# ishine/usdm

Hardware: AMD Instinct MI355X
Metric: end-to-end real-time factor + LLM tokens/sec, 10 s utterance, 7B TP=1/8 (higher is better)
Workload: dtype bf16; 1 GPU; full pipeline, one 10 s utterance: XLS-R tokenizer -> Mistral-7B (3 greedy rounds) -> Token-Voicebox 63 NFE (Heun, CFG, 3 s prompt) -> BigVGAN; wave_samples=160000, mel_frames=861, output_samples=220416, parallelism=tp1 (LLM) + replicas, tp_comm=none, voicebox=replica (CFG batch 2 on every rank)

## Files before the change

### include/usdm_hip.h

```cpp
#ifndef USDM_HIP_H_
#define USDM_HIP_H_
#include <stdint.h>

#ifdef __cplusplus
extern "C" {
#endif

typedef void* usdm_stream_t;

enum { USDM_BF16 = 0, USDM_F32 = 1 };
enum { USDM_ACT_NONE = 0, USDM_ACT_GELU = 1, USDM_ACT_SWIGLU = 3, USDM_ACT_TANH = 4, USDM_ACT_LOGCLAMP = 5  };
enum { USDM_EPI_PLAIN = 0, USDM_EPI_QKV_HEADS = 1 };

const char* usdm_last_error(void);
int usdm_abi_version(void);

typedef struct usdm_gemm_args {
  int32_t dtype;
  int32_t M, N;
  int32_t taps, Kc;
  const void* A;
  int64_t lda;
  int32_t rowsA;
  int32_t a_row_mul, a_row_off, a_row_step;
// ... 177 lines not shown
int usdm_sizeof_gemv_mxfp4_args(void);

typedef struct usdm_gemv_mxfp4_mfma_args {
  usdm_gemv_batch_args b;
  const void* codes;
  int64_t ldc;
  const uint8_t* scales;
  int64_t lds;
} usdm_gemv_mxfp4_mfma_args;
int usdm_gemv_mxfp4_mfma(const usdm_gemv_mxfp4_mfma_args* args, usdm_stream_t stream);
int usdm_sizeof_gemv_mxfp4_mfma_args(void);

typedef struct usdm_gemv_wpack {
  const void* planes;
  const uint8_t* rowflag;
  int64_t stride;
  int32_t base;
  int32_t units;
  uint32_t marked[448];
} usdm_gemv_wpack;
int usdm_gemv_packed(const usdm_gemv_args* args, const usdm_gemv_wpack* pack, usdm_stream_t stream);
int usdm_gemv_packs(const usdm_gemv_args* args);
int usdm_sizeof_gemv_wpack(void);

typedef struct usdm_decode_state {
  int32_t* next_token;
  int32_t* out_tokens;
  int32_t* step;
  int32_t* pos;
  int32_t max_out, id_offset, advance_pos;
  int32_t batch;
  int32_t* done; const int32_t* eos;
} usdm_decode_state;
int usdm_argmax_final(const float* part_val, const int32_t* part_idx, int32_t nparts,
                      const usdm_decode_state* st, const void* embed_table_bf16, int32_t Hd, void* h_out_bf16,
                      usdm_stream_t stream);
int usdm_argmax_final_seg(const float* part_val, const int32_t* part_idx, int32_t nparts, int32_t nseg, int64_t seg_stride,
                          const usdm_decode_state* st, const void* embed_table, int32_t Hd, void* h_out, usdm_stream_t stream);

typedef struct usdm_sample_params {
  float temperature; int32_t top_k; float top_p;
  float min_p;
  uint64_t seed;
} usdm_sample_params;
typedef struct usdm_sample_args {
  const float* logits; int32_t V;
// ... 244 lines not shown
```

### usdm_amd/_lib.py

```python
import ctypes as C
import os

_HERE = os.path.dirname(os.path.abspath(__file__))
LIB_PATH = os.path.join(_HERE, "libusdm_hip.so")


class UsdmError(RuntimeError):
    pass


if not os.path.exists(LIB_PATH):
    raise ImportError(
        f"{LIB_PATH} not found: build it with `python -m usdm_amd.build` (hipcc --offload-arch=gfx950). "
        "usdm_amd has no CPU fallback.")

lib = C.CDLL(LIB_PATH, mode=C.RTLD_GLOBAL)
lib.usdm_last_error.restype = C.c_char_p
lib.usdm_gemv_batch_ks_floats.restype = C.c_int64
lib.usdm_gemm_tile_info.restype = C.c_int
lib.usdm_gemv_fp8_mfma.restype = C.c_int
lib.usdm_attn_decode_fp8.restype = C.c_int
lib.usdm_rope_cache_fp8.restype = C.c_int
lib.usdm_gemv_mxfp4.restype = C.c_int
lib.usdm_dequant_mxfp4.restype = C.c_int
lib.usdm_gemv_mxfp4_mfma.restype = C.c_int
lib.usdm_gemv_packed.restype = C.c_int
lib.usdm_gemv_packs.restype = C.c_int
lib.usdm_logprobs.restype = C.c_int
lib.usdm_logprobs_seg.restype = C.c_int
lib.usdm_prompt_logprobs.restype = C.c_int
lib.usdm_prompt_logprobs_seg.restype = C.c_int
lib.usdm_penalize.restype = C.c_int
lib.usdm_penalize_seg.restype = C.c_int
lib.usdm_penalty_params_init.restype = C.c_int
lib.usdm_logit_edit.restype = C.c_int
lib.usdm_logit_edit_seg.restype = C.c_int
lib.usdm_beam_step.restype = C.c_int
lib.usdm_kv_reorder.restype = C.c_int
lib.usdm_kv_expand.restype = C.c_int
lib.usdm_attn_verify.restype = C.c_int
lib.usdm_spec_commit.restype = C.c_int
lib.usdm_attn_verify_batch.restype = C.c_int
lib.usdm_spec_commit_batch.restype = C.c_int
_exp = None


def exp():
    global _exp
    if _exp is None:
        path = os.path.join(_HERE, "libusdm_hip_experimental.so")
# ... 313 lines not shown
```

### usdm_amd/csrc/llm_k.hip

```cpp
#include "common.h"
#include <stdlib.h>
#include <utility>
#include "../../include/usdm_hip.h"
#include "gemv_launch.h"
#include "gemv_pieces.h"
#include "attn_merge.h"
#include "p2p.h"
#include "pick_commit.h"

#ifndef USDM_GEMV_DOWN_UNR
#define USDM_GEMV_DOWN_UNR 8
#endif
#ifndef USDM_GEMV_WPACK_RU
#define USDM_GEMV_WPACK_RU 3
#endif
#ifndef USDM_GEMV_WPACK_UB
#define USDM_GEMV_WPACK_UB 12
#endif
namespace {
#ifdef USDM_GEMV_TRACE
__device__ unsigned long long g_gemv_trace[8192 * 8];
#define GTR(i) do { if (threadIdx.x == 0 && blockIdx.x < 8192) g_gemv_trace[blockIdx.x * 8 + (i)] = wall_clock64(); } while (0)
#else
#define GTR(i) do { } while (0)
#endif


template <int RW, bool GLU, int NWV, bool MRG = false, bool P2P = false, bool CMB = false, bool FP8 = false, class... FMT>
__global__ __launch_bounds__(NWV * 64) void gemv_kernel(const usdm_gemv_args a, FMT... fmt) {
  typedef typename gemv_fmt<FP8>::wvec wvec;
  constexpr bool MX4 = gemv_is_mx4<FMT...>::value;
  static_assert((FP8 || MX4) == (sizeof...(FMT) == 1) && !(FP8 && MX4), "FP8 takes the row exponents, MXFP4 the block scales");
  static_assert(!(FP8 || MX4) || (!MRG && !P2P && !CMB), "the FP8 / MXFP4 weight formats have the plain single-GPU forms only");
  constexpr int NTH = NWV * 64;
  constexpr int NR = GLU ? 2 * RW : RW;
  constexpr int UNR = gemv_ring_depth(NR, FP8, MX4);
  extern __shared__ __attribute__((aligned(16))) char smem[];
  bf16_t* xs = (bf16_t*)smem;
  __shared__ float red[NWV];
  __shared__ float sv[NWV];
// ... 606 lines not shown
    gemv_for<NU>([&](auto UI) {
      constexpr int un = decltype(UI)::value, s = un % RU;
      constexpr int younger = un + RU < NU ? 4 * (RU - 1) : 4 * (NU - 1 - un);
      gemv_wunit& r = ring[s];
      asm volatile("s_waitcnt vmcnt(%4)" : "+v"(r.la), "+v"(r.lb), "+v"(r.nib), "+v"(r.sgn) : "n"(younger) : "memory");
      gemv_for<4>([&](auto PI) {
        constexpr int P = decltype(PI)::value, it = 4 * un + P;
        const u32x4 xn = *(const u32x4*)(xs + (((it + 1) % NIT) * 64 + lane) * 8);
        const u32x4& lo = P < 2 ? r.la : r.lb;
        acc = dot8(gemv_wpack8<P>(lo[2 * (P & 1)], lo[2 * (P & 1) + 1], r.nib[P], r.sgn, base4), xv, acc);
        xv = xn;
      });
      if constexpr (un + RU < NU) gemv_unit_load<un + RU>(r, pp, voff);
    });
  }
  acc = wave_sum(acc);

  if (lane != 0 || ob >= a.N) return;
  const float v = gemv_plain_value(acc, a.round_bf16, a.residual != nullptr, [&] { return bf2f(resraw); });
  if (a.y16) ((bf16_t*)a.y16)[ob] = f2bf(v);
  if (a.y32) a.y32[ob] = v;
}

__global__ void argmax_final_kernel(const float* pv, const int* pi, int nparts, int nseg, int64_t seg_stride, usdm_decode_state st,
                                    const bf16_t* E, int Hd, bf16_t* h_out) {
  __shared__ float sv[256];
  __shared__ int si[256];
  __shared__ int s_tok;
  const int b = blockIdx.x;
  if (st.done && st.done[b]) return;
  pv += (int64_t)b * nparts; pi += (int64_t)b * nparts;
  float bv = -INFINITY;
  int bi = PICK_NO_ID;
  for (int sg = 0; sg < nseg; ++sg)
    for (int i = threadIdx.x; i < nparts; i += 256) {
      const float v = pv[sg * seg_stride + i];
      const int id = pi[sg * seg_stride + i];
      if (pick_better(v, id, bv, bi)) { bv = v; bi = id; }
    }
  pick_block_best<256>(sv, si, bv, bi);
  if (threadIdx.x == 0) {
    const int tok = (si[0] == PICK_NO_ID ? 0 : si[0]) + st.id_offset;
    pick_commit(st, b, st.step[b], tok);
    s_tok = tok;
  }
  if (E) {
    __syncthreads();
    pick_embed_row<256>(E, s_tok, Hd, h_out + (int64_t)b * Hd);
  }
}

__global__ void embed_kernel(const bf16_t* E, const int64_t* ids, const int* next_token, int n, int Hd, bf16_t* out) {
  const int r = blockIdx.x;
  const int64_t id = ids ? ids[r] : (int64_t)(*next_token);
  const u32x4* src = (const u32x4*)(E + id * Hd);
  u32x4* dst = (u32x4*)(out + (int64_t)r * Hd);
  for (int i = threadIdx.x; i < Hd / 8; i += blockDim.x) dst[i] = src[i];
}

__global__ void residual_add_kernel(bf16_t* h, const float* delta, int n) {
  const int i = blockIdx.x * blockDim.x + threadIdx.x;
  if (i < n) h[i] = f2bf(bf2f(h[i]) + round_bf(delta[i]));
}
}

static int gemv_resident_count(const void* kern, int nth, size_t lds, int* out) {
  static thread_local const void* c_kern = nullptr;
  static thread_local int c_dev = -1, c_n = 0;
  static thread_local size_t c_lds = 0;
  int dev = 0;
  USDM_HIP(hipGetDevice(&dev));
  if (kern != c_kern || dev != c_dev || lds != c_lds) {
    int ncu = 0, per = 0;
    USDM_HIP(hipDeviceGetAttribute(&ncu, hipDeviceAttributeMultiprocessorCount, dev));
    USDM_HIP(hipOccupancyMaxActiveBlocksPerMultiprocessor(&per, kern, nth, lds));
    USDM_CHECK_ARG(ncu > 0 && per > 0, "usdm_gemv: the resident form does not fit a CU (%zu bytes of LDS)", lds);
    c_kern = kern; c_dev = dev; c_lds = lds; c_n = ncu * per;
  }
  *out = c_n;
  return 0;
}

static int gemv_launch_resident(const usdm_gemv_args& a, const gemv_sel& s, size_t lds, hipStream_t st, bool* launched) {
  *launched = false;
  if (a.x_delta) return 0;
  constexpr int RW = 2, NWV = 7;
  auto straight = gemv_resident_kernel<RW, NWV, 2, 8>;
  auto generic = gemv_resident_kernel<RW, NWV, 0, 0>;
  const int ntiles = s.grid;
  int n = 0;
  if (int rc = gemv_resident_count((const void*)straight, NWV * 64, lds, &n)) return rc;
  int grid = min(min(n, s.res), ntiles);
  if (grid == ntiles) return 0;
  if (a.K == 8 * 512 && ntiles == 2 * grid) {
    hipLaunchKernelGGL(straight, dim3(grid), dim3(NWV * 64), lds, st, a);
  } else {
    if (int rc = gemv_resident_count((const void*)generic, NWV * 64, lds, &n)) return rc;
    grid = min(min(n, s.res), ntiles);
    if (grid == ntiles) return 0;
    hipLaunchKernelGGL(generic, dim3(grid), dim3(NWV * 64), lds, st, a);
  }
  *launched = true;
  USDM_LAUNCH_CHECK();
  return 0;
}

template <int FORM, bool MRG, bool P2P, bool CMB, bool FP8, class... FMT>
static int gemv_launch(const usdm_gemv_args& a, hipStream_t st, FMT... fmt) {
  const size_t lds = (size_t)((a.K + 511) & ~511) * 2;
  const gemv_sel s = gemv_select(a, false);
  if constexpr (FORM == GEMV_PLAIN && !FP8 && sizeof...(FMT) == 0) {
    if (s.stream) {
      hipLaunchKernelGGL((gemv_stream_kernel<28, USDM_GEMV_DOWN_UNR>), dim3(s.grid), dim3(1024), lds, st, a);
      USDM_LAUNCH_CHECK();
      return 0;
    }
    if (s.res > 0) {
// ... 41 lines not shown
  }
  return gemv_launch<GEMV_PLAIN, false, false, false, false>(a, st);
}

extern "C" int usdm_gemv_packs(const usdm_gemv_args* pa) { return gemv_select(*pa, false).stream ? 1 : 0; }

extern "C" int usdm_gemv_packed(const usdm_gemv_args* pa, const usdm_gemv_wpack* pk, usdm_stream_t stream) {
  USDM_CHECK_ARG(pa && pa->W && pa->x && pk && pk->planes && pk->rowflag, "usdm_gemv_packed: null args");
  USDM_CHECK_ARG(pa->N <= 14336, "usdm_gemv_packed: at most 14336 rows (usdm_gemv_wpack.marked)");
  if (!usdm_gemv_packs(pa)) return usdm_gemv(pa, stream);
  const usdm_gemv_args& a = *pa;
  if (int rc = gemv_check_shape("usdm_gemv_packed", a, "input vector")) return rc;
  if (int rc = gemv_check_outputs("usdm_gemv_packed", a)) return rc;
  USDM_CHECK_ARG(pk->units == 7 && pk->units * 2048 == a.K && pk->stride % 16 == 0 && pk->stride >= (int64_t)pk->units * GEMV_WPACK_UNIT &&
                     pk->base >= 0 && pk->base <= 112,
                 "usdm_gemv_packed: the image must hold K / 2048 units of 3328 bytes per row, stride a multiple of 16, base 0..112");
  USDM_CHECK_ARG(((uintptr_t)pk->planes & 15) == 0 && ((uintptr_t)pk->rowflag & 3) == 0, "usdm_gemv_packed: planes must be 16-byte, rowflag 4-byte aligned");
  const gemv_sel s = gemv_select(a, false);
  hipLaunchKernelGGL((gemv_stream_wpack_kernel<28, USDM_GEMV_WPACK_RU, USDM_GEMV_WPACK_UB>), dim3(s.grid), dim3(1024), (size_t)a.K * 2,
                     (hipStream_t)stream, a, *pk);
  USDM_LAUNCH_CHECK();
  return 0;
}
extern "C" int usdm_sizeof_gemv_wpack(void) { return (int)sizeof(usdm_gemv_wpack); }

int usdm_gemv_fp8_batch_launch(const usdm_gemv_fp8_args* pa, hipStream_t st);

extern "C" int usdm_gemv_fp8(const usdm_gemv_fp8_args* pa, usdm_stream_t stream) {
  USDM_CHECK_ARG(pa && pa->b.g.W && pa->b.g.x && pa->row_exp, "usdm_gemv_fp8: null args");
  const usdm_gemv_args& a = pa->b.g;
  USDM_CHECK_ARG(pa->b.nb >= 1 && pa->b.nb <= 4 && (pa->b.form == 0 || pa->b.form == -1),
                 "usdm_gemv_fp8: 1..4 sequences on the VALU form (the matrix-core form has no FP8 weights)");
  USDM_CHECK_ARG(!a.p2p && !a.p2p_mode && !a.mrg_po && !a.cmb_gran && !a.x_delta && !a.x_out,
                 "usdm_gemv_fp8: p2p / merged-attention input / cmb_gran / x_delta are not supported with FP8 weights");
  USDM_CHECK_ARG(((uintptr_t)a.W & 7) == 0, "usdm_gemv_fp8: bad N/K/ldw");
  if (int rc = gemv_check_shape("usdm_gemv_fp8", a, "input vector")) return rc;
  if (int rc = gemv_check_outputs("usdm_gemv_fp8", a)) return rc;
  hipStream_t st = (hipStream_t)stream;
  if (pa->b.nb > 1) return usdm_gemv_fp8_batch_launch(pa, st);
  return gemv_launch<GEMV_PLAIN, false, false, false, true>(a, st, pa->row_exp);
}

namespace {
__global__ __launch_bounds__(256) void dequant_fp8_kernel(const uint8_t* q, const int8_t* row_exp, int K, int64_t ldq, bf16_t* out,
                                                          int64_t ldo) {
  const int r = blockIdx.x;
// ... 128 lines not shown
```

### usdm_amd/llm.py

```python
import math
import os
import time
from collections import namedtuple

import torch

from . import ops
from ._lib import ACT_SWIGLU, UsdmError
from .graph import GraphedPlan, GraphedSegments
from .plancache import LRU
from .prefix import reusable_past
from .quant import Fp8Weight, Mxfp4Weight, check_kv_cache_dtype
from .wpack import PackedWeight
from .slots import (CHUNK, NO_CANDIDATE_IDX, BeamSlots, DecodeSlots, SpecSequence, SpecSlots, TokenLogprobs, edit_buffers, logprob_buffers,
                    penalty_buffers, read_logprobs, seed_edits, seed_penalties, stop_block, stop_index)

MISTRAL_7B_USDM = dict(vocab_size=42003, hidden_size=4096, intermediate_size=14336, num_hidden_layers=32,
                       num_attention_heads=32, num_key_value_heads=8, head_dim=128, rms_norm_eps=1e-5,
                       rope_theta=10000.0, max_position_embeddings=32768)


def _pack_gate_up(gate, up):
    I, K = gate.shape
    return torch.stack([gate.reshape(I // 16, 16, K), up.reshape(I // 16, 16, K)], 1).reshape(2 * I, K).contiguous()
# ... 139 lines not shown
         "lm_head": qz_head(g("lm_head.weight")[v0:v1].contiguous()), "layers": [], "v0": v0, "v1": v1}
    for l in range(cfg["num_hidden_layers"]):
        p = f"model.layers.{l}."
        q = g(p + "self_attn.q_proj.weight")[rank * Hq * d:(rank + 1) * Hq * d]
        k = g(p + "self_attn.k_proj.weight")[rank * Hkv * d:(rank + 1) * Hkv * d]
        v = g(p + "self_attn.v_proj.weight")[rank * Hkv * d:(rank + 1) * Hkv * d]
        o = g(p + "self_attn.o_proj.weight")[:, rank * Hq * d:(rank + 1) * Hq * d]
        ga = g(p + "mlp.gate_proj.weight")[rank * I:(rank + 1) * I]
        up = g(p + "mlp.up_proj.weight")[rank * I:(rank + 1) * I]
        dn = g(p + "mlp.down_proj.weight")[:, rank * I:(rank + 1) * I]
        W["layers"].append(dict(qkv=qz(torch.cat([q, k, v], 0).contiguous()), o=qz(o.contiguous()), gu=qz(_pack_gate_up(ga, up)),
                                down=qz(dn.contiguous()), ln1=f(p + "input_layernorm.weight"),
                                ln2=f(p + "post_attention_layernorm.weight")))
        del q, k, v, o, ga, up, dn
    return W


class USDMForCausalLM:
    def __init__(self, cfg, device, ctx_max=2048, tp_rank=0, tp_size=1, group=None, decode_splits=None, tp_segments=None, p2p=None,
                 p2p_fused=None, quantization=None, fp8_matrix_cores=False, kv_cache_dtype=None, score_rows=256,
                 enable_prefix_caching=False, weight_packing=None, mxfp4_matrix_cores=False):
        check_quantization(quantization, fp8_matrix_cores, mxfp4_matrix_cores)
        self.weight_packing = (os.environ.get("USDM_WPACK", "1") != "0") if weight_packing is None else bool(weight_packing)
        self.wpack_report = None
        self.prefix_caching = bool(enable_prefix_caching)
        if self.prefix_caching:
            if tp_size > 1 or tp_segments or p2p is not None:
                raise NotImplementedError("enable_prefix_caching runs on one GPU: tensor parallelism (tp_size > 1, tp_segments, p2p) is not supported")
            if os.environ.get("USDM_PREFIX_REUSE", "exact") in ("0", "off"):
                raise ValueError("enable_prefix_caching=True contradicts USDM_PREFIX_REUSE=0 (prefix reuse switched off)")
        if isinstance(score_rows, bool) or not isinstance(score_rows, int) or score_rows < 16 or score_rows % 16:
            raise ValueError(f"score_rows must be a positive multiple of 16, got {score_rows!r}")
        self.score_rows = score_rows
        if quantization is not None and (tp_size > 1 or tp_segments or p2p is not None):
            raise NotImplementedError(f"quantization={quantization!r} runs on one GPU: tensor parallelism (tp_size > 1, tp_segments, p2p) takes bf16 weights")
        self.kv_cache_dtype = check_kv_cache_dtype(kv_cache_dtype)
        self.kv8 = self.kv_cache_dtype == "fp8"
        if self.kv8 and (tp_size > 1 or tp_segments or p2p is not None):
            raise NotImplementedError("kv_cache_dtype='fp8' runs on one GPU: tensor parallelism (tp_size > 1, tp_segments, p2p) takes a bf16 cache")
        if self.kv8 and os.environ.get("USDM_GEMV_CHAIN", "0") not in ("", "0"):
            raise NotImplementedError("kv_cache_dtype='fp8': the chained decode GEMVs (USDM_GEMV_CHAIN) take a bf16 cache")
        self.quantization = quantization
        self.fp8_matrix_cores = bool(fp8_matrix_cores)
        self.mxfp4_matrix_cores = bool(mxfp4_matrix_cores)
        self.cfg = dict(cfg)
        self.device = torch.device(device)
# ... 127 lines not shown
                           p + "mlp.gate_proj.weight": ((I, H), H ** -0.5), p + "mlp.up_proj.weight": ((I, H), H ** -0.5),
                           p + "mlp.down_proj.weight": ((H, I), I ** -0.5)})

        def get(n):
            if n.endswith("norm.weight") or n.endswith("layernorm.weight"):
                return torch.ones(H, device=m.device)
            shape, sc = shapes[n]
            return (torch.randn(shape, device=m.device, dtype=torch.float32, generator=gen) * sc).to(torch.bfloat16)
        m.W = m._shard(get)
        m._alloc()
        return m

    def weight_bytes_per_token(self):
        if self.quantization is not None:
            return sum(l[k].nbytes for l in self.W["layers"] for k in QUANT_KEYS) + self.W["lm_head"].nbytes
        n = sum(l[k].numel() for l in self.W["layers"] for k in ("qkv", "o", "gu", "down")) + self.W["lm_head"].numel()
        return 2 * n

    def kv_bytes_per_token_row(self):
        d = self.cfg["head_dim"]
        return 2 * self.cfg["num_hidden_layers"] * self.Hkv * ((d + 1) if self.kv8 else 2 * d)

    def _pack_weights(self):
        self.wpack_down = None
        if not (self.weight_packing and self.tp_size == 1 and not self.tp_path and self.p2p is None and self.quantization is None
                and self.cfg["hidden_size"] == 4096 and self.I == 14336):
            return
        t0 = time.perf_counter()
        self.wpack_down = [PackedWeight.from_matrix(w["down"]) for w in self.W["layers"]]
        torch.cuda.synchronize(self.device)
        self.wpack_report = {"down_marked_share": [p.marked_share for p in self.wpack_down],
                             "down_marked_rows": sum(len(p.marked_rows) for p in self.wpack_down),
                             "extra_bytes": sum(p.nbytes for p in self.wpack_down), "seconds": time.perf_counter() - t0}

    def _alloc(self):
        self._pack_weights()
        c, dev = self.cfg, self.device
        L, d = c["num_hidden_layers"], c["head_dim"]
        bf = torch.bfloat16
        if self.kv8:
            self.kcache = torch.zeros(L, self.Hkv, self.ctx_max, d, dtype=torch.uint8, device=dev)
            self.vcache = torch.zeros(L, self.Hkv, self.ctx_max, d, dtype=torch.uint8, device=dev)
            self.kexp = torch.zeros(L, self.Hkv, self.ctx_max, dtype=torch.int8, device=dev)
            self.vexp = torch.zeros(L, self.Hkv, self.ctx_max, dtype=torch.int8, device=dev)
        else:
            self.kcache = torch.zeros(L, self.Hkv, self.ctx_max, d, dtype=bf, device=dev)
            self.vcache = torch.zeros(L, self.Hkv, self.ctx_max, d, dtype=bf, device=dev)
        mode = os.environ.get("USDM_PREFIX_REUSE", "exact")
        self.reuse_prefix = {"0": False, "off": False, "1": True, "all": True}.get(mode, "exact")
        if self.kv8:
            self.vtc = None
            if not self.prefix_caching:
                self.reuse_prefix = False
        else:
            self.vtc = torch.zeros(L, self.Hkv, d, self.ctx_max, dtype=bf, device=dev)
        self._kv_ids, self._vt_upto = None, 0
# ... 149 lines not shown
                ops.penalize(logits, st, V=self.v1 - self.v0, plan=rec.plan, **pen)
            if sampling == "hook":
                rec.cut(lambda: self.logits_hook())
            ops.sample_final(logits, st, dev_params=sl.sample_params, plan=rec.plan, **out)
            if lp:
                ops.logprobs(logits, st, V=self.v1 - self.v0, plan=rec.plan, **lp)
        elif p2p is not None:
            site = 2 * c["num_hidden_layers"]
            self._p2p_exchange(rec, st, lambda ph: ops.argmax_p2p(sl.part_val_loc, sl.part_idx_loc, self.nparts, st, p2p, site, phase=ph,
                                                                  plan=rec.plan, **out))
        else:
            if self.tp_path:
                rec.cut(self._gather_partials if single else
                        (lambda: self._gather_partials([sl.part_val, sl.part_idx], [sl.part_val_loc, sl.part_idx_loc])))
            seg = dict(nseg=self.tp_size, seg_stride=B * self.nparts) if (B and self.tp_path) else {}
            ops.argmax_final(sl.part_val, sl.part_idx, self.nparts * (1 if B else self.tp_size), st, plan=rec.plan, **seg, **out)
        rec.plan.hold(st)

    def _dims(self):
        c = self.cfg
        H, d = c["hidden_size"], c["head_dim"]
        return H, d, c["num_hidden_layers"], self.Hq, self.Hkv, self.I, (self.Hq + 2 * self.Hkv) * d

    def _layers(self, rec, gemv, attn, h, qkv, ao, act, way, n=0, parts=None, h_alt=None, down_kw={}, down_wp=None):
        H, d, _, Hq, Hkv, I, nq = self._dims()
        eps, h0, pend = self.cfg["rms_norm_eps"], h, None

        def proj(W, ln, N, out, a=0):
            nonlocal h, pend
            if pend is None:
                return gemv(W, h, N=N, K=H, norm_w=ln, eps=eps, act=a, y16=out)
            nxt = h_alt if h is h0 else h0
            gemv(W, h, N=N, K=H, norm_w=ln, eps=eps, act=a, y16=out, x_delta=pend, x_out=nxt)
            h, pend = nxt, None

        def land(W, x, K, site, **kw):
            nonlocal pend
            if way == "fused":
                return gemv(W, x, N=H, K=K, residual=h, y16=h, **kw)
            if way == "p2p":
                mode = 1 if self.p2p_fused else 2
                gemv(W, x, N=H, K=K, residual=h, y16=h, p2p=self.p2p, p2p_site=site, p2p_mode=mode, **kw)
                rec.cut()
                if mode == 2:
                    ops.p2p_reduce(self.p2p, site, H, h, skip=self.st_done, plan=rec.plan)
                return
            part = parts[site & 1]
            gemv(W, x, N=H, K=K, round_bf16=False, y32=part, **kw)
            rec.cut(lambda: self._all_reduce(part))
            if way == "deferred":
                pend = part
            else:
                ops.residual_add(h, part, n, plan=rec.plan)

        for l, w in enumerate(self.W["layers"]):
            proj(w["qkv"], w["ln1"], nq, qkv)
            o_kw = attn(l) or {}
            land(w["o"], ao, Hq * d, 2 * l, **o_kw)
            proj(w["gu"], w["ln2"], 2 * I, act, ACT_SWIGLU)
            land(w["down"], act, I, 2 * l + 1, **down_kw, **({"wpack": down_wp[l]} if down_wp else {}))
        return h, pend

    def _prefill_rows(self, S, slot=None, past=0):
        dev, bf = self.device, torch.bfloat16
        H, d, L, Hq, Hkv, I, nq = self._dims()
        scratch = slot is not None or self.kv8
        Spad = ((past if scratch else 0) + S + 63) // 64 * 64
        rec = _Segments()
        Z = lambda *s, dt=bf: rec.plan.hold(torch.zeros(*s, device=dev, dtype=dt))
        io = dict(ids=Z(S, dt=torch.int64))
        h, xn, qkv, ao, act = Z(S, H), Z(S, H), Z(S, nq), Z(S, Hq * d), Z(S, I)
        vt = Z(Hkv, d, Spad) if scratch else None
        kscr = Z(Hkv, Spad, d) if self.kv8 else None
        part = Z(S, H, dt=torch.float32) if self.tp_path else None
        ops.embed_rows(self.W["embed"], h, Hd=H, ids=io["ids"], n=S, plan=rec.plan)

        def gemm(W, x, *, N, K, norm_w=None, eps=None, act=0, residual=None, y16=None, y32=None, round_bf16=True):
            if norm_w is not None:
                ops.norm(x, norm_w, None, rows=S, C=H, eps=eps, rms=True, round_bf16=True, out16=xn, plan=rec.plan)
                x = xn
            ops.gemm(x, self._gemm_w(W, rec.plan), M=S, N=N, Kc=K, act=act, round_bf16=round_bf16 and (bool(act) or residual is not None),
                     residual=residual, ldr=H if residual is not None else 0, out32=y32, out16=y16, ldc=N // 2 if act else N, plan=rec.plan)
# ... 97 lines not shown
            else:
                ops.gemv_chain(chain, sync, plan=rec.plan)
            chain = None

        def gemv(W, x, **kw):
            if chain is None:
                return ops.gemv(W, x, skip=skp, plan=rec.plan, **kw)
            chain.append(ops.gemv(W, x, skip=skp, only_args=True, **kw))
            if len(chain) == self.chain:
                flush()

        def attn(l):
            nonlocal chain
            gran = cmb_gran[l] if use_cmb else None
            ops.attn_decode(qkv, self.st_pos, self.cos, self.sin, self.kcache[l], self.vcache[l], pm, pl, po, ao, Hq=Hq, Hkv=Hkv,
                            ctx_max=self.ctx_max, NS=self.NS, scale=d ** -0.5, counters=cnt, skip=skp, defer_merge=mrg is not None, window=self.window,
                            cmb_gran=gran, kv8=(self.kexp[l], self.vexp[l]) if self.kv8 else None, plan=rec.plan)
            if chained:
                chain = []
                return None
            return dict(merge=mrg, cmb=(gran, self.cmb_err) if use_cmb else None)

        h, pend = self._layers(rec, gemv, attn, h, qkv, ao, act, way, n=H, parts=parts, h_alt=h_alt,
                               down_wp=self.wpack_down if way == "fused" else None)
        if chain:
            flush()
        self._lm_head_and_pick(rec, h, True, sampling, x_delta=pend, skip=skp, logprobs=logprobs, penalties=penalties, edits=edits)
        return rec.finish()

    @staticmethod
    def _run_segs(segs):
        for s in segs:
            if isinstance(s, ops.Plan):
                s.run()
            else:
                s()

    def _graphed(self, built, enabled=None):
        segs = built if isinstance(built, list) else [built]
        if any(not isinstance(s, ops.Plan) for s in segs):
            return GraphedSegments(segs, self._run_segs, enabled=enabled)
        plan = segs[0]
        if len(segs) > 1:
            plan = ops.Plan()
            for s in segs:
                plan.calls += s.calls
                plan.hold(*s.keep)
# ... 510 lines not shown
```

### usdm_amd/ops.py

```python
import ctypes as C_
import os

import torch

from . import _lib
from ._lib import (BF16, F32, AttnVerifyArgs, AttnVerifyBatchArgs, SpecArgs, SpecBatchArgs, BeamArgs, KvExpandArgs, KvReorderArgs, AttnArgs, AttnDecodeArgs, AttnDecodeFp8Args, RopeFp8Args, DecodeState, GemmArgs, GemvArgs, GemvBatchArgs, GemvFp8Args, GemvMxfp4Args, GemvMxfp4MfmaArgs, LogitEditArgs, LogprobArgs, NormArgs, PenaltyArgs, PromptLogprobArgs, RopeArgs, SampleArgs, SnakeArgs,
                   VbInputArgs, VbSolverArgs, check, lib)
from .quant import Fp8Weight, Mxfp4Weight
from .wpack import GemvWpack

if lib.usdm_sizeof_gemv_wpack() != C_.sizeof(GemvWpack):
    raise ImportError(f"ABI mismatch: usdm_gemv_wpack is {lib.usdm_sizeof_gemv_wpack()} bytes in the library, {C_.sizeof(GemvWpack)} in Python")


def _stream():
    return C_.c_void_p(torch.cuda.current_stream().cuda_stream)


class Plan:

    def __init__(self):
        self.calls = []
        self.keep = []

# ... 229 lines not shown
    if cmb is not None:
        gran, err = cmb
        _need_cuda(gran, err)
        if merge is None or gran.numel() * gran.element_size() < (a.K // 2) * 8:
            raise ValueError("usdm_gemv: cmb needs merge=(pm, pl, po, NS) and K/2 8-byte granules")
        a.cmb_gran, a.cmb_err, a.cmb_timeout_ms = _ptr(gran), _ptr(err), 200
    if p2p is not None and p2p_mode:
        p2p.check_site(p2p_site, a.N)
        a.p2p, a.p2p_site, a.p2p_mode = p2p.dev_ptr, p2p_site, p2p_mode
    if isinstance(W, Fp8Weight):
        if only_args:
            raise ValueError("usdm_gemv: FP8 weights have no chained form")
        f = GemvFp8Args()
        f.b.g, f.b.nb, f.row_exp = a, 1, _ptr(W.e)
        _go(plan, "usdm_gemv_fp8", lib.usdm_gemv_fp8, C_.byref(f))
        return
    if isinstance(W, Mxfp4Weight):
        if only_args:
            raise ValueError("usdm_gemv: MXFP4 weights have no chained form")
        f = GemvMxfp4Args()
        f.b.g, f.b.nb, f.scales, f.lds = a, 1, _ptr(W.s), W.s.shape[1]
        _go(plan, "usdm_gemv_mxfp4", lib.usdm_gemv_mxfp4, C_.byref(f))
        return
    if wpack is not None and not only_args and lib.usdm_gemv_packs(C_.byref(a)):
        if not wpack.is_cuda or (wpack.N, wpack.K) != (a.N, a.K):
            raise ValueError("usdm_gemv: wpack is the image of another matrix")
        p = wpack.args()
        if plan is not None:
            plan.hold(wpack.planes, wpack.rowflag)
        _go(plan, "usdm_gemv", lib.usdm_gemv_packed, C_.byref(a), C_.byref(p))
        return
    if only_args:
        return a
    _go(plan, "usdm_gemv", lib.usdm_gemv, C_.byref(a))


def gemv_engine(phases, sync, gran, timeout_ms=2000, plan=None):
    _need_cuda(sync, gran)
    if not (1 <= len(phases) <= 4) or sync.numel() < 8 or sync.element_size() != 4 or gran.numel() * gran.element_size() < 3 * 8192 * 8:
        raise ValueError("gemv_engine: 1..4 phases, an 8-word sync block and 192 KB of granule space")
    c = _lib.GemvChainArgs()
    for i, ph in enumerate(phases):
        c.ph[i] = ph
    c.nph, c.sync, c.timeout_ms, c.gran = len(phases), _ptr(sync), timeout_ms, _ptr(gran)
    _go(plan, "usdm_gemv_engine", _lib.exp().usdm_gemv_engine, C_.byref(c))


def gemv_chain(phases, sync, timeout_ms=2000, plan=None):
    _need_cuda(sync)
    if not (1 <= len(phases) <= 4) or sync.numel() < 8 or sync.element_size() != 4:
        raise ValueError("gemv_chain: 1..4 phases and an 8-word sync block")
    c = _lib.GemvChainArgs()
    for i, ph in enumerate(phases):
# ... 559 lines not shown
```

### usdm_amd/wpack.py

```python
import ctypes as C

import torch

UNIT_ELEMS = 2048
UNIT_BYTES = 3328
MAX_ROWS = 14336


def _i16(w):
    if w.dtype != torch.bfloat16 or w.dim() != 2 or w.shape[1] % UNIT_ELEMS:
        raise ValueError("wpack: a bf16 [N][K] matrix with K a multiple of 2048")
    return w.contiguous().view(torch.int16).to(torch.int32) & 0xffff


def _pick_base(e7):
    rmin, rmax = e7.amin(dim=1), e7.amax(dim=1)
    cand = torch.arange(0, 0x7f - 15 + 1, device=e7.device)
    fits = ((rmin[None, :] >= cand[:, None]) & (rmax[None, :] <= cand[:, None] + 15)).sum(dim=1)
    best = int(fits.max().item())
    return int(cand[fits == best].min().item())


def pack(w):
    b = _i16(w)
    N, K = b.shape
    U = K // UNIT_ELEMS
    e7 = (b >> 8) & 0x7f
    base = _pick_base(e7)
    idx = e7 - base
# ... 16 lines not shown


def unpack(planes, base, K):
    N, U = planes.shape[0], K // UNIT_ELEMS
    p = planes.view(N, U, UNIT_BYTES).to(torch.int32)
    low = torch.cat((p[..., :1024].reshape(N, U, 64, 16), p[..., 1024:2048].reshape(N, U, 64, 16)), dim=3)
    lo = low.view(N, U, 64, 4, 8).permute(0, 1, 3, 2, 4)
    nb = p[..., 2048:3072].reshape(N, U, 64, 4, 4).permute(0, 1, 3, 2, 4)
    ix = torch.cat((nb & 15, nb >> 4), dim=4)
    sb = p[..., 3072:].reshape(N, U, 64, 4).to(torch.int64)
    sd = (sb[..., 0] | (sb[..., 1] << 8) | (sb[..., 2] << 16) | (sb[..., 3] << 24)).view(N, U, 1, 64, 1)
    i_ = torch.arange(4, device=planes.device).view(4, 1, 1)
    k_ = torch.arange(8, device=planes.device).view(1, 1, 8)
    sg = ((sd >> (8 * (k_ & 3) + 7 - (2 * i_ + (k_ >> 2)))) & 1).to(torch.int32)
    return (lo | ((ix + base) << 8) | (sg << 15)).reshape(N, K)


class GemvWpack(C.Structure):
    _fields_ = [("planes", C.c_void_p), ("rowflag", C.c_void_p), ("stride", C.c_int64), ("base", C.c_int32), ("units", C.c_int32),
                ("marked", C.c_uint32 * (MAX_ROWS // 32))]


class PackedWeight:
    __slots__ = ("planes", "rowflag", "base", "N", "K", "marked_rows")

    def __init__(self, planes, rowflag, base, K):
        self.planes, self.rowflag, self.base, self.K = planes, rowflag, int(base), K
        self.N = planes.shape[0]
        if self.N > MAX_ROWS:
            raise ValueError(f"wpack: at most {MAX_ROWS} rows")
        self.marked_rows = torch.nonzero(rowflag[:self.N]).flatten().tolist()

    @classmethod
    def from_matrix(cls, w):
        planes, flag, base = pack(w)
        ok = (unpack(planes, base, w.shape[1]) == _i16(w)).all(dim=1) | (flag[:w.shape[0]] != 0)
        if not bool(ok.all()):
            raise RuntimeError("wpack: the packed image does not reproduce the matrix")
        return cls(planes, flag, base, w.shape[1])

    @property
    def is_cuda(self):
        return self.planes.is_cuda

    @property
    def marked_share(self):
        return len(self.marked_rows) / self.N

    @property
    def nbytes(self):
        return self.planes.numel() + self.rowflag.numel()

    def args(self):
        a = GemvWpack()
        a.planes, a.rowflag = C.c_void_p(self.planes.data_ptr()), C.c_void_p(self.rowflag.data_ptr())
        a.stride, a.base, a.units = self.planes.shape[1], self.base, self.K // UNIT_ELEMS
        for r in self.marked_rows:
            a.marked[r >> 5] |= 1 << (r & 31)
        return a
```

Before: 5.557 x real-time (output audio s / wall s).

## Extend lossless exponent-packed weight image to the fused gate/up SwiGLU GEMV

```diff
diff --git a/include/usdm_hip.h b/include/usdm_hip.h
--- a/include/usdm_hip.h
+++ b/include/usdm_hip.h
@@ -223,6 +223,8 @@
 int usdm_gemv_packed(const usdm_gemv_args* args, const usdm_gemv_wpack* pack, usdm_stream_t stream);
 int usdm_gemv_packs(const usdm_gemv_args* args);
 int usdm_sizeof_gemv_wpack(void);
+int usdm_gemv_packed_glu(const usdm_gemv_args* args, const usdm_gemv_wpack* pack, usdm_stream_t stream);
+int usdm_gemv_packs_glu(const usdm_gemv_args* args);
 
 typedef struct usdm_decode_state {
   int32_t* next_token;
diff --git a/usdm_amd/_lib.py b/usdm_amd/_lib.py
--- a/usdm_amd/_lib.py
+++ b/usdm_amd/_lib.py
@@ -26,6 +26,8 @@
 lib.usdm_gemv_mxfp4_mfma.restype = C.c_int
 lib.usdm_gemv_packed.restype = C.c_int
 lib.usdm_gemv_packs.restype = C.c_int
+lib.usdm_gemv_packed_glu.restype = C.c_int
+lib.usdm_gemv_packs_glu.restype = C.c_int
 lib.usdm_logprobs.restype = C.c_int
 lib.usdm_logprobs_seg.restype = C.c_int
 lib.usdm_prompt_logprobs.restype = C.c_int
diff --git a/usdm_amd/csrc/llm_k.hip b/usdm_amd/csrc/llm_k.hip
--- a/usdm_amd/csrc/llm_k.hip
+++ b/usdm_amd/csrc/llm_k.hip
@@ -16,6 +16,9 @@
 #endif
 #ifndef USDM_GEMV_WPACK_UB
 #define USDM_GEMV_WPACK_UB 12
+#endif
+#ifndef USDM_GEMV_GU_WPACK_RU
+#define USDM_GEMV_GU_WPACK_RU 4
 #endif
 namespace {
 #ifdef USDM_GEMV_TRACE
@@ -668,6 +671,159 @@
   if (a.y32) a.y32[ob] = v;
 }
 
+template <int RU>
+__global__ __launch_bounds__(7 * 64) __attribute__((amdgpu_waves_per_eu(4))) void gemv_resident_wpack_kernel(const usdm_gemv_args a,
+                                                                                                          const usdm_gemv_wpack p) {
+  constexpr int RW = 2, NWV = 7, TPW = 2, NIT = 8;
+  constexpr int NTH = NWV * 64, NR = 2 * RW, TILE = NWV * RW;
+  constexpr int UNR = gemv_ring_depth(NR, false, false);
+  constexpr int NU = NIT / 4, NSEQ = TPW * NU * NR;
+  static_assert(RU >= 1 && RU <= NSEQ && NIT >= UNR && NIT % UNR == 0, "a full first ring; slot u = iteration u of every tile");
+  extern __shared__ __attribute__((aligned(16))) char smem[];
+  bf16_t* xs = (bf16_t*)smem;
+  __shared__ float red[NWV];
+  const int tid = threadIdx.x, lane = tid & 63, wave = tid >> 6;
+  const int skipv = a.skip ? *a.skip : 0;
+  const int K = a.K;
+  const int Kpad = (K + 511) & ~511;
+  const int uwave = __builtin_amdgcn_readfirstlane(wave);
+  auto row_of = [&](int t, int j) -> int {
+    const int r = gemv_glu_row((blockIdx.x + t * gridDim.x) * TILE + uwave * RW + (j % RW), j >= RW);
+    return r < a.N ? r : a.N - 1;
+  };
+  unsigned mk = 0u;
+#pragma unroll
+  for (int t = 0; t < TPW; ++t) {
+    const int o = (blockIdx.x + t * gridDim.x) * TILE + uwave * RW;
+    if (2 * o < a.N) mk |= (p.marked[o >> 5] >> (o & 31)) & 3u;
+  }
+  const unsigned voff = lane * 16;
+  const int i0 = tid * 8;
+  auto stage = [&](u32x4 x0, u32x4 ge0v, u32x4 ge1v) {
+    const float4 ge0 = __builtin_bit_cast(float4, ge0v), ge1 = __builtin_bit_cast(float4, ge1v);
+    const bf16_t* xg = (const bf16_t*)a.x;
+    const int iloop = i0 + NTH * 8;
+    if (a.norm_w) {
+      float ss = 0.f;
+      if (i0 < K) ss = gemv_sumsq8(x0, ss);
+      for (int i = iloop; i < K; i += NTH * 8) ss = gemv_sumsq8(*(const u32x4*)(xg + i), ss);
+      const float rstd = gemv_rms_rstd<NWV>(ss, red, K, a.eps);
+      if (i0 < Kpad) *(u32x4*)(xs + i0) = i0 < K ? gemv_rmsnorm8(x0, rstd, ge0, ge1) : u32x4{0, 0, 0, 0};
+      for (int i = iloop; i < Kpad; i += NTH * 8) {
+        u32x4 o = {0, 0, 0, 0};
+        if (i < K) o = gemv_rmsnorm8(*(const u32x4*)(xg + i), rstd, *(const float4*)(a.norm_w + i), *(const float4*)(a.norm_w + i + 4));
+        *(u32x4*)(xs + i) = o;
+      }
+    } else {
+      if (i0 < Kpad) *(u32x4*)(xs + i0) = i0 < K ? x0 : u32x4{0, 0, 0, 0};
+      for (int i = iloop; i < Kpad; i += NTH * 8) {
+        u32x4 v = {0, 0, 0, 0};
+        if (i < K) v = *(const u32x4*)(xg + i);
+        *(u32x4*)(xs + i) = v;
+      }
+    }
+    __syncthreads();
+  };
+  auto finish = [&](int t, float (&acc)[NR]) {
+#pragma unroll
+    for (int j = 0; j < NR; ++j) acc[j] = wave_sum(acc[j]);
+    if (lane == 0) {
+      const int ob = (blockIdx.x + t * gridDim.x) * TILE + wave * RW;
+#pragma unroll
+      for (int j = 0; j < RW; ++j) {
+        const int o = ob + j;
+        if (2 * o >= a.N) continue;
+        const float r = gemv_swiglu_value(acc[j], acc[j + RW], a.round_bf16);
+        if (a.y16) ((bf16_t*)a.y16)[o] = f2bf(r);
+        if (a.y32) a.y32[o] = r;
+      }
+    }
+  };
+  float acc[NR];
+  if (mk) {
+    const char* wp[NR];
+    const char* wn[NR];
+#pragma unroll
+    for (int j = 0; j < NR; ++j) wp[j] = (const char*)((const bf16_t*)a.W + (int64_t)row_of(0, j) * a.ldw);
+    u32x4 x0 = {0u, 0u, 0u, 0u}, ge0v = x0, ge1v = x0;
+    gemv_early_loads(a, i0, K, x0, ge0v, ge1v);
+    u32x4 ring[NR][UNR];
+    gemv_for<UNR>([&](auto U) { gemv_for<NR>([&](auto J) { gemv_ring_load<U.value>(ring[J.value][U.value], wp[J.value], voff); }); });
+    asm volatile("s_waitcnt vmcnt(%3)" : "+v"(x0), "+v"(ge0v), "+v"(ge1v) : "n"(UNR * NR));
+    if (skipv) return;
+    stage(x0, ge0v, ge1v);
+    u32x4 xv = *(const u32x4*)(xs + lane * 8);
+    gemv_for<TPW>([&](auto T) {
+      constexpr int t = decltype(T)::value;
+      constexpr bool has_next = t + 1 < TPW;
+#pragma unroll
+      for (int j = 0; j < NR; ++j) {
+        acc[j] = 0.f;
+        wn[j] = has_next ? (const char*)((const bf16_t*)a.W + (int64_t)row_of(t + 1, j) * a.ldw) : wp[j];
+      }
+      gemv_for<NIT>([&](auto IT) {
+        constexpr int it = decltype(IT)::value, u = it % UNR;
+        constexpr bool refill = it + UNR < NIT || has_next;
+        const u32x4 xn = *(const u32x4*)(xs + (((it + 1) % NIT) * 64 + lane) * 8);
+        gemv_for<NR>([&](auto J) {
+          constexpr int j = decltype(J)::value;
+          constexpr int younger = refill ? NR * UNR - 1 : NR * UNR - 1 - ((it - (NIT - UNR)) * NR + j);
+          asm volatile("s_waitcnt vmcnt(%1)" : "+v"(ring[j][u]) : "n"(younger) : "memory");
+          acc[j] = dot8(ring[j][u], xv, acc[j]);
+          if constexpr (it + UNR < NIT) gemv_ring_load<it + UNR>(ring[j][u], wp[j], voff);
+          else if constexpr (has_next) gemv_ring_load<u>(ring[j][u], wn[j], voff);
+        });
+        xv = xn;
+      });
+      finish(t, acc);
+#pragma unroll
+      for (int j = 0; j < NR; ++j) wp[j] = wn[j];
+    });
+  } else {
+    const char* pp[TPW][NR];
+#pragma unroll
+    for (int t = 0; t < TPW; ++t)
+#pragma unroll
+      for (int j = 0; j < NR; ++j) pp[t][j] = (const char*)p.planes + (int64_t)row_of(t, j) * p.stride;
+    const unsigned base4 = (unsigned)p.base * 0x01010101u;
+    u32x4 x0 = {0u, 0u, 0u, 0u}, ge0v = x0, ge1v = x0;
+    gemv_early_loads(a, i0, K, x0, ge0v, ge1v);
+    gemv_wunit ring[RU];
+    gemv_for<RU>([&](auto S) {
+      constexpr int s = decltype(S)::value;
+      gemv_unit_load<(s / NR) % NU>(ring[s], pp[s / (NR * NU)][s % NR], voff);
+    });
+    asm volatile("s_waitcnt vmcnt(%3)" : "+v"(x0), "+v"(ge0v), "+v"(ge1v) : "n"(4 * RU));
+    if (skipv) return;
+    stage(x0, ge0v, ge1v);
+    u32x4 xq[4];
+#pragma unroll
+    for (int P = 0; P < 4; ++P) xq[P] = *(const u32x4*)(xs + (P * 64 + lane) * 8);
+    gemv_for<TPW>([&](auto T) {
+      constexpr int t = decltype(T)::value;
+#pragma unroll
+      for (int j = 0; j < NR; ++j) acc[j] = 0.f;
+      gemv_for<NU>([&](auto UI) {
+        constexpr int un = decltype(UI)::value;
+        gemv_for<NR>([&](auto J) {
+          constexpr int j = decltype(J)::value, s = (t * NU + un) * NR + j, s2 = s + RU;
+          constexpr int younger = s2 < NSEQ ? 4 * (RU - 1) : 4 * (NSEQ - 1 - s);
+          gemv_wunit& r = ring[s % RU];
+          asm volatile("s_waitcnt vmcnt(%4)" : "+v"(r.la), "+v"(r.lb), "+v"(r.nib), "+v"(r.sgn) : "n"(younger) : "memory");
+          gemv_for<4>([&](auto PI) {
+            constexpr int P = decltype(PI)::value;
+            const u32x4& lo = P < 2 ? r.la : r.lb;
+            acc[j] = dot8(gemv_wpack8<P>(lo[2 * (P & 1)], lo[2 * (P & 1) + 1], r.nib[P], r.sgn, base4), xq[P], acc[j]);
+            if constexpr (j == NR - 1) xq[P] = *(const u32x4*)(xs + ((4 * ((un + 1) % NU) + P) * 64 + lane) * 8);
+          });
+          if constexpr (s2 < NSEQ) gemv_unit_load<(s2 / NR) % NU>(r, pp[s2 / (NR * NU)][s2 % NR], voff);
+        });
+      });
+      finish(t, acc);
+    });
+  }
+}
+
 __global__ void argmax_final_kernel(const float* pv, const int* pi, int nparts, int nseg, int64_t seg_stride, usdm_decode_state st,
                                     const bf16_t* E, int Hd, bf16_t* h_out) {
   __shared__ float sv[256];
@@ -710,6 +866,7 @@
 }
 }
 
+template <int WHO = 0>
 static int gemv_resident_count(const void* kern, int nth, size_t lds, int* out) {
   static thread_local const void* c_kern = nullptr;
   static thread_local int c_dev = -1, c_n = 0;
@@ -727,6 +884,10 @@
   return 0;
 }
 
+static bool gemv_straight_form(const usdm_gemv_args& a, int ntiles, int grid) {
+  return !a.x_delta && a.K == 8 * 512 && ntiles == 2 * grid;
+}
+
 static int gemv_launch_resident(const usdm_gemv_args& a, const gemv_sel& s, size_t lds, hipStream_t st, bool* launched) {
   *launched = false;
   if (a.x_delta) return 0;
@@ -738,7 +899,7 @@
   if (int rc = gemv_resident_count((const void*)straight, NWV * 64, lds, &n)) return rc;
   int grid = min(min(n, s.res), ntiles);
   if (grid == ntiles) return 0;
-  if (a.K == 8 * 512 && ntiles == 2 * grid) {
+  if (gemv_straight_form(a, ntiles, grid)) {
     hipLaunchKernelGGL(straight, dim3(grid), dim3(NWV * 64), lds, st, a);
   } else {
     if (int rc = gemv_resident_count((const void*)generic, NWV * 64, lds, &n)) return rc;
@@ -826,6 +987,39 @@
   USDM_LAUNCH_CHECK();
   return 0;
 }
+static int gemv_packed_glu_grid(const usdm_gemv_args& a, int* grid) {
+  *grid = 0;
+  const gemv_sel s = gemv_select(a, false);
+  if (!(s.glu && s.rw == 2 && s.nwv == 7 && s.res > 0) || a.x_out || a.K != 8 * 512 || a.x_delta) return 0;
+  int n = 0;
+  if (int rc = gemv_resident_count<1>((const void*)gemv_resident_wpack_kernel<USDM_GEMV_GU_WPACK_RU>, 7 * 64, (size_t)a.K * 2, &n)) return rc;
+  const int g = min(min(n, s.res), s.grid);
+  if (gemv_straight_form(a, s.grid, g)) *grid = g;
+  return 0;
+}
+
+extern "C" int usdm_gemv_packs_glu(const usdm_gemv_args* pa) {
+  int grid = 0;
+  return pa && gemv_packed_glu_grid(*pa, &grid) == 0 && grid > 0 ? 1 : 0;
+}
+
+extern "C" int usdm_gemv_packed_glu(const usdm_gemv_args* pa, const usdm_gemv_wpack* pk, usdm_stream_t stream) {
+  USDM_CHECK_ARG(pa && pa->W && pa->x && pk && pk->planes && pk->rowflag, "usdm_gemv_packed_glu: null args");
+  USDM_CHECK_ARG(pa->act == USDM_ACT_SWIGLU && pa->N / 2 <= 14336, "usdm_gemv_packed_glu: a SwiGLU call of at most 14336 outputs (usdm_gemv_wpack.marked)");
+  const usdm_gemv_args& a = *pa;
+  int grid = 0;
+  if (int rc = gemv_packed_glu_grid(a, &grid)) return rc;
+  if (!grid) return usdm_gemv(pa, stream);
+  if (int rc = gemv_check_shape("usdm_gemv_packed_glu", a, "input vector")) return rc;
+  if (int rc = gemv_check_outputs("usdm_gemv_packed_glu", a)) return rc;
+  USDM_CHECK_ARG(pk->units == 2 && pk->stride % 16 == 0 && pk->stride >= (int64_t)2 * GEMV_WPACK_UNIT && pk->base >= 0 && pk->base <= 112,
+                 "usdm_gemv_packed_glu: the image must hold 2 units of 3328 bytes per row, stride a multiple of 16, base 0..112");
+  USDM_CHECK_ARG(((uintptr_t)pk->planes & 15) == 0 && ((uintptr_t)pk->rowflag & 3) == 0,
+                 "usdm_gemv_packed_glu: planes must be 16-byte, rowflag 4-byte aligned");
+  hipLaunchKernelGGL((gemv_resident_wpack_kernel<USDM_GEMV_GU_WPACK_RU>), dim3(grid), dim3(7 * 64), (size_t)a.K * 2, (hipStream_t)stream, a, *pk);
+  USDM_LAUNCH_CHECK();
+  return 0;
+}
 extern "C" int usdm_sizeof_gemv_wpack(void) { return (int)sizeof(usdm_gemv_wpack); }
 
 int usdm_gemv_fp8_batch_launch(const usdm_gemv_fp8_args* pa, hipStream_t st);
diff --git a/usdm_amd/llm.py b/usdm_amd/llm.py
--- a/usdm_amd/llm.py
+++ b/usdm_amd/llm.py
@@ -185,6 +185,7 @@
                  enable_prefix_caching=False, weight_packing=None, mxfp4_matrix_cores=False):
         check_quantization(quantization, fp8_matrix_cores, mxfp4_matrix_cores)
         self.weight_packing = (os.environ.get("USDM_WPACK", "1") != "0") if weight_packing is None else bool(weight_packing)
+        self.weight_packing_gu = self.weight_packing and os.environ.get("USDM_WPACK_GU", "1") != "0"
         self.wpack_report = None
         self.prefix_caching = bool(enable_prefix_caching)
         if self.prefix_caching:
@@ -358,7 +359,7 @@
         return 2 * self.cfg["num_hidden_layers"] * self.Hkv * ((d + 1) if self.kv8 else 2 * d)
 
     def _pack_weights(self):
-        self.wpack_down = None
+        self.wpack_down = self.wpack_gu = None
         if not (self.weight_packing and self.tp_size == 1 and not self.tp_path and self.p2p is None and self.quantization is None
                 and self.cfg["hidden_size"] == 4096 and self.I == 14336):
             return
@@ -368,6 +369,12 @@
         self.wpack_report = {"down_marked_share": [p.marked_share for p in self.wpack_down],
                              "down_marked_rows": sum(len(p.marked_rows) for p in self.wpack_down),
                              "extra_bytes": sum(p.nbytes for p in self.wpack_down), "seconds": time.perf_counter() - t0}
+        if self.weight_packing_gu:
+            t0 = time.perf_counter()
+            self.wpack_gu = [PackedWeight.from_matrix(w["gu"], glu=True) for w in self.W["layers"]]
+            torch.cuda.synchronize(self.device)
+            self.wpack_report.update({"gu_marked_outputs": [len(p.marked_outputs) for p in self.wpack_gu],
+                                      "gu_extra_bytes": sum(p.nbytes for p in self.wpack_gu), "gu_seconds": time.perf_counter() - t0})
 
     def _alloc(self):
         self._pack_weights()
@@ -563,16 +570,16 @@
         H, d = c["hidden_size"], c["head_dim"]
         return H, d, c["num_hidden_layers"], self.Hq, self.Hkv, self.I, (self.Hq + 2 * self.Hkv) * d
 
-    def _layers(self, rec, gemv, attn, h, qkv, ao, act, way, n=0, parts=None, h_alt=None, down_kw={}, down_wp=None):
+    def _layers(self, rec, gemv, attn, h, qkv, ao, act, way, n=0, parts=None, h_alt=None, down_kw={}, down_wp=None, gu_wp=None):
         H, d, _, Hq, Hkv, I, nq = self._dims()
         eps, h0, pend = self.cfg["rms_norm_eps"], h, None
 
-        def proj(W, ln, N, out, a=0):
+        def proj(W, ln, N, out, a=0, **kw):
             nonlocal h, pend
             if pend is None:
-                return gemv(W, h, N=N, K=H, norm_w=ln, eps=eps, act=a, y16=out)
+                return gemv(W, h, N=N, K=H, norm_w=ln, eps=eps, act=a, y16=out, **kw)
             nxt = h_alt if h is h0 else h0
-            gemv(W, h, N=N, K=H, norm_w=ln, eps=eps, act=a, y16=out, x_delta=pend, x_out=nxt)
+            gemv(W, h, N=N, K=H, norm_w=ln, eps=eps, act=a, y16=out, x_delta=pend, x_out=nxt, **kw)
             h, pend = nxt, None
 
         def land(W, x, K, site, **kw):
@@ -598,7 +605,7 @@
             proj(w["qkv"], w["ln1"], nq, qkv)
             o_kw = attn(l) or {}
             land(w["o"], ao, Hq * d, 2 * l, **o_kw)
-            proj(w["gu"], w["ln2"], 2 * I, act, ACT_SWIGLU)
+            proj(w["gu"], w["ln2"], 2 * I, act, ACT_SWIGLU, **({"wpack": gu_wp[l]} if gu_wp else {}))
             land(w["down"], act, I, 2 * l + 1, **down_kw, **({"wpack": down_wp[l]} if down_wp else {}))
         return h, pend
 
@@ -742,7 +749,7 @@
             return dict(merge=mrg, cmb=(gran, self.cmb_err) if use_cmb else None)
 
         h, pend = self._layers(rec, gemv, attn, h, qkv, ao, act, way, n=H, parts=parts, h_alt=h_alt,
-                               down_wp=self.wpack_down if way == "fused" else None)
+                               down_wp=self.wpack_down if way == "fused" else None, gu_wp=self.wpack_gu if way == "fused" else None)
         if chain:
             flush()
         self._lm_head_and_pick(rec, h, True, sampling, x_delta=pend, skip=skp, logprobs=logprobs, penalties=penalties, edits=edits)
diff --git a/usdm_amd/ops.py b/usdm_amd/ops.py
--- a/usdm_amd/ops.py
+++ b/usdm_amd/ops.py
@@ -275,13 +275,15 @@
         f.b.g, f.b.nb, f.scales, f.lds = a, 1, _ptr(W.s), W.s.shape[1]
         _go(plan, "usdm_gemv_mxfp4", lib.usdm_gemv_mxfp4, C_.byref(f))
         return
-    if wpack is not None and not only_args and lib.usdm_gemv_packs(C_.byref(a)):
-        if not wpack.is_cuda or (wpack.N, wpack.K) != (a.N, a.K):
+    glu = a.act == _lib.ACT_SWIGLU
+    packs, packed = (lib.usdm_gemv_packs_glu, lib.usdm_gemv_packed_glu) if glu else (lib.usdm_gemv_packs, lib.usdm_gemv_packed)
+    if wpack is not None and not only_args and packs(C_.byref(a)):
+        if not wpack.is_cuda or (wpack.N, wpack.K, wpack.glu) != (a.N, a.K, glu):
             raise ValueError("usdm_gemv: wpack is the image of another matrix")
         p = wpack.args()
         if plan is not None:
             plan.hold(wpack.planes, wpack.rowflag)
-        _go(plan, "usdm_gemv", lib.usdm_gemv_packed, C_.byref(a), C_.byref(p))
+        _go(plan, "usdm_gemv", packed, C_.byref(a), C_.byref(p))
         return
     if only_args:
         return a
diff --git a/usdm_amd/wpack.py b/usdm_amd/wpack.py
--- a/usdm_amd/wpack.py
+++ b/usdm_amd/wpack.py
@@ -5,6 +5,10 @@
 UNIT_ELEMS = 2048
 UNIT_BYTES = 3328
 MAX_ROWS = 14336
+
+
+def glu_row(o, up):
+    return (o >> 4) * 32 + (o & 15) + (16 if up else 0)
 
 
 def _i16(w):
@@ -67,22 +71,25 @@
 
 
 class PackedWeight:
-    __slots__ = ("planes", "rowflag", "base", "N", "K", "marked_rows")
+    __slots__ = ("planes", "rowflag", "base", "N", "K", "marked_rows", "glu", "marked_outputs")
 
-    def __init__(self, planes, rowflag, base, K):
-        self.planes, self.rowflag, self.base, self.K = planes, rowflag, int(base), K
+    def __init__(self, planes, rowflag, base, K, glu=False):
+        self.planes, self.rowflag, self.base, self.K, self.glu = planes, rowflag, int(base), K, bool(glu)
         self.N = planes.shape[0]
-        if self.N > MAX_ROWS:
-            raise ValueError(f"wpack: at most {MAX_ROWS} rows")
+        if glu and self.N % 32:
+            raise ValueError("wpack: a gate/up matrix has a multiple of 32 rows")
+        if (self.N // 2 if glu else self.N) > MAX_ROWS:
+            raise ValueError(f"wpack: at most {MAX_ROWS} {'outputs' if glu else 'rows'}")
         self.marked_rows = torch.nonzero(rowflag[:self.N]).flatten().tolist()
+        self.marked_outputs = torch.nonzero(rowflag[:self.N].view(-1, 2, 16).amax(dim=1).flatten()).flatten().tolist() if glu else None
 
     @classmethod
-    def from_matrix(cls, w):
+    def from_matrix(cls, w, glu=False):
         planes, flag, base = pack(w)
         ok = (unpack(planes, base, w.shape[1]) == _i16(w)).all(dim=1) | (flag[:w.shape[0]] != 0)
         if not bool(ok.all()):
             raise RuntimeError("wpack: the packed image does not reproduce the matrix")
-        return cls(planes, flag, base, w.shape[1])
+        return cls(planes, flag, base, w.shape[1], glu)
 
     @property
     def is_cuda(self):
@@ -100,6 +107,6 @@
         a = GemvWpack()
         a.planes, a.rowflag = C.c_void_p(self.planes.data_ptr()), C.c_void_p(self.rowflag.data_ptr())
         a.stride, a.base, a.units = self.planes.shape[1], self.base, self.K // UNIT_ELEMS
-        for r in self.marked_rows:
+        for r in (self.marked_outputs if self.glu else self.marked_rows):
             a.marked[r >> 5] |= 1 << (r & 31)
         return a
```

After: 5.858 x real-time (output audio s / wall s), median of 6. +5.4%, better.
